# AnyLoc/Revisit-Anything

Measured on AMD Instinct MI355X. Metric: query_images_per_sec, higher is better.
Workload: dtype f32

## Files before the change

### revisit-anything_amd/csrc/api.hip

```cpp
#include <stdarg.h>
#include <stdlib.h>
#include <string.h>

#include <cmath>
#include <mutex>
#include <utility>

#include <initializer_list>

#include "ctx.h"

int segvlad_ctx::fail(int code, const char* fmt, ...) {
  va_list ap;
  va_start(ap, fmt);
  vsnprintf(err, sizeof(err), fmt, ap);
  va_end(ap);
  return code;
}

bool sv_is_device_ptr(const void* p) {
  hipPointerAttribute_t a;
  memset(&a, 0, sizeof(a));
  hipError_t e = hipPointerGetAttributes(&a, p);
  if (e != hipSuccess) {
// ... 97 lines not shown

int sv_fork_side(segvlad_ctx* ctx) {
  if (!ctx->side) {
    SV_HIP(hipStreamCreateWithFlags(&ctx->side, hipStreamNonBlocking));
    SV_HIP(hipEventCreateWithFlags(&ctx->ev_fork, hipEventDisableTiming));
    SV_HIP(hipEventCreateWithFlags(&ctx->ev_join, hipEventDisableTiming));
  }
  SV_HIP(hipEventRecord(ctx->ev_fork, ctx->stream));
  SV_HIP(hipStreamWaitEvent(ctx->side, ctx->ev_fork, 0));
  return SEGVLAD_OK;
}

int sv_join_side(segvlad_ctx* ctx) {
  SV_HIP(hipEventRecord(ctx->ev_join, ctx->side));
  SV_HIP(hipStreamWaitEvent(ctx->stream, ctx->ev_join, 0));
  return SEGVLAD_OK;
}

int sv_guard_check(segvlad_ctx* ctx) {
  if (!ctx->guard) return SEGVLAD_OK;
  SV_HIP(hipDeviceSynchronize());
  if (!ctx->guard_hit[0]) {
    ctx->for_each_buf([&](DevBuf& b) {
      if (!b.raw || ctx->guard_hit[0]) return;
      const int front = guard_words_hit(b.raw), back = guard_words_hit(static_cast<unsigned char*>(b.p) + b.fence_off());
      if (front)
        snprintf(ctx->guard_hit, sizeof(ctx->guard_hit), "%s: %d words written BELOW the buffer", b.tag, front);
      else if (back)
        snprintf(ctx->guard_hit, sizeof(ctx->guard_hit), "%s: %d words written beyond the %zu bytes requested", b.tag, back, b.fixed ? b.cap : b.req);
    });
  }
  if (ctx->guard_hit[0]) return ctx->fail(SEGVLAD_ERR_STATE, "guard: out-of-bounds write, buffer %s", ctx->guard_hit);
  return SEGVLAD_OK;
}

StageTimer* sv_stage_open(segvlad_ctx* c, const char* name, int* slot) {
  if (!c->profiling || c->scope_mute) return nullptr;
  StageTimer* t = &c->timers[name];
  if (t->used * 2 >= (int)t->ev.size()) {
    hipEvent_t a = nullptr, b = nullptr;
    (void)hipEventCreate(&a);
    (void)hipEventCreate(&b);
    t->ev.push_back(a);
    t->ev.push_back(b);
  }
  *slot = t->used++;
  (void)hipEventRecord(t->ev[2 * *slot], c->stream);
  return t;
}

hipError_t sv_max_dyn_lds(const void* fn, size_t bytes) {
  static std::mutex mu;
  static std::map<std::pair<int, const void*>, size_t> done;
  int dev = 0;
  hipError_t e = hipGetDevice(&dev);
  if (e != hipSuccess) return e;
  std::lock_guard<std::mutex> lk(mu);
  auto it = done.find({dev, fn});
  if (it != done.end() && it->second >= bytes) return hipSuccess;
  e = hipFuncSetAttribute(fn, hipFuncAttributeMaxDynamicSharedMemorySize, (int)bytes);
  if (e == hipSuccess) done[{dev, fn}] = bytes;
  return e;
}

extern "C" {

int segvlad_version(void) { return 300; }

int segvlad_create(segvlad_ctx** out, int device_id) {
  if (!out) return SEGVLAD_ERR_ARG;
  *out = nullptr;
  int ndev = 0;
  if (hipGetDeviceCount(&ndev) != hipSuccess || device_id < 0 || device_id >= ndev) return SEGVLAD_ERR_HIP;
  if (hipSetDevice(device_id) != hipSuccess) return SEGVLAD_ERR_HIP;
  segvlad_ctx* c = new (std::nothrow) segvlad_ctx();
  if (!c) return SEGVLAD_ERR_NOMEM;
  c->device = device_id;
  static const char* const env_keys[][2] = {{"SEGVLAD_KNN_FILTER", "knn_filter"},   {"SEGVLAD_F16_CFG", "f16_cfg"},
                                            {"SEGVLAD_F16_GM", "f16_gm"},           {"SEGVLAD_X3_TILE", "x3_tile"},
                                            {"SEGVLAD_X3_GM", "x3_gm"},             {"SEGVLAD_SEARCH_STATS", "search_stats"},
                                            {"SEGVLAD_ASSIGN_NARROW", "assign_narrow"}, {"SEGVLAD_DEBUG_SEARCH", "debug_search"},
                                            {"SEGVLAD_AGG_KPB", "agg_kpb"},
                                            {"SEGVLAD_KNN_HEURISTIC", "knn_heuristic"}, {"SEGVLAD_PCA_PATH", "pca_path"},
                                            {"SEGVLAD_COVER_ROWS", "cover_rows"}};
  for (auto& kv : env_keys)
    if (const char* v = getenv(kv[0])) (void)segvlad_set_option(c, kv[1], v);
#define SV_TAG_P(n) c->n.tag = #n; c->n.fixed = true;
#define SV_TAG_S(n) c->n.tag = #n;
  SV_PERSISTENT_BUFS(SV_TAG_P)
  SV_SCRATCH_BUFS(SV_TAG_S)
#undef SV_TAG_P
#undef SV_TAG_S
  if (const char* v = getenv("SEGVLAD_GUARD")) {
    if (v[0] && v[0] != '0') {
      c->guard = true;
      c->for_each_buf([](DevBuf& b) { b.guard = true; });
    }
  }
  if (const char* v = getenv("SEGVLAD_RCCL_LIB")) snprintf(sv_rccl_lib_override, sizeof(sv_rccl_lib_override), "%s", v);
  if (getenv("SEGVLAD_KNN_FP32")) (void)segvlad_set_option(c, "knn_filter", "fp32");
  if (getenv("SEGVLAD_PCA_FP32")) (void)segvlad_set_option(c, "pca_arith", "fp32");
  c->err[0] = 0;
  *out = c;
  return SEGVLAD_OK;
}

int segvlad_set_option(segvlad_ctx* ctx, const char* key, const char* value) {
  if (!ctx) return SEGVLAD_ERR_ARG;
  if (!key || !value) return ctx->fail(SEGVLAD_ERR_ARG, "set_option: null key/value");
  SvOptions& o = ctx->opt;
  auto as_int = [&](int* dst) -> int {
    char* end = nullptr;
    const long v = strtol(value, &end, 10);
    if (end == value || *end) return ctx->fail(SEGVLAD_ERR_ARG, "set_option(%s): '%s' is not an integer", key, value);
    *dst = (int)v;
    return SEGVLAD_OK;
  };
  if (!strcmp(key, "knn_filter")) {
    if (!strcmp(value, "auto")) o.knn_filter = 0;
    else if (!strcmp(value, "f16")) o.knn_filter = 1;
    else if (!strcmp(value, "bf16x3")) o.knn_filter = 2;
    else if (!strcmp(value, "fp32")) o.knn_filter = 3;
    else return ctx->fail(SEGVLAD_ERR_ARG, "set_option(knn_filter): want auto|f16|bf16x3|fp32, got '%s'", value);
    return SEGVLAD_OK;
  }
  if (!strcmp(key, "pca_arith")) {
    if (!strcmp(value, "auto") || !strcmp(value, "f16x3")) o.pca_fp32 = 0;
    else if (!strcmp(value, "fp32")) o.pca_fp32 = 1;
    else return ctx->fail(SEGVLAD_ERR_ARG, "set_option(pca_arith): want auto|f16x3|fp32, got '%s'", value);
    return SEGVLAD_OK;
  }
  if (!strcmp(key, "pca_path")) {
    if (!strcmp(value, "auto")) o.pca_path = 0;
    else if (!strcmp(value, "planes")) o.pca_path = 1;
    else if (!strcmp(value, "project")) o.pca_path = 2;
    else return ctx->fail(SEGVLAD_ERR_ARG, "set_option(pca_path): want auto|planes|project, got '%s'", value);
    return SEGVLAD_OK;
  }
  if (!strcmp(key, "vlad_assign")) {
    if (!strcmp(value, "hard")) {
      o.vlad_soft_temp = 0.f, o.vlad_soft_pooled = 0;
      return SEGVLAD_OK;
    }
    const int pooled = !strncmp(value, "soft_pooled:", 12);
    if (pooled || !strncmp(value, "soft:", 5)) {
      const char* t = value + (pooled ? 12 : 5);
      bool decimal = *t != 0 && (*t == '.' || (*t >= '0' && *t <= '9'));
      for (const char* c = t; *c && decimal; ++c) decimal = strchr("0123456789.eE+-", *c) != nullptr;
      char* end = nullptr;
      const float temp = decimal ? strtof(t, &end) : 0.f;
      if (decimal && end != t && *end == 0 && std::isfinite(temp) && temp > 0.f) {
        o.vlad_soft_temp = temp, o.vlad_soft_pooled = pooled;
        return SEGVLAD_OK;
      }
    }
    return ctx->fail(SEGVLAD_ERR_ARG, "set_option(vlad_assign): want hard|soft:<T>|soft_pooled:<T> with a finite decimal T > 0, got '%s'", value);
  }
  if (!strcmp(key, "vlad_burst")) {
    if (!strcmp(value, "off")) {
      o.vlad_burst = 0, o.burst_a = o.burst_b = o.burst_p = 0.f;
      return SEGVLAD_OK;
    }
    static const float lo[3] = {0.f, -8.f, 0.f}, hi[3] = {64.f, 16.f, 2.f};
    float v[3] = {0.f, 0.f, 0.f};
    const char* t = value;
    bool ok = true;
    for (int f = 0; f < 3 && ok; ++f) {
      const char* stop = f < 2 ? strchr(t, ':') : t + strlen(t);
      ok = stop != nullptr && stop != t && (*t == '.' || *t == '-' || (*t >= '0' && *t <= '9'));
      for (const char* c = t; ok && c < stop; ++c) ok = strchr("0123456789.eE+-", *c) != nullptr;
      if (!ok) break;
      char* end = nullptr;
      v[f] = strtof(t, &end);
      ok = end == stop && std::isfinite(v[f]) && v[f] >= lo[f] && v[f] <= hi[f];
      t = stop + 1;
    }
    if (ok) {
      o.vlad_burst = 1, o.burst_a = v[0], o.burst_b = v[1], o.burst_p = v[2];
      return SEGVLAD_OK;
    }
    return ctx->fail(SEGVLAD_ERR_ARG, "set_option(vlad_burst): want off|<a>:<b>:<p>, finite decimals with 0 <= a <= 64, -8 <= b <= 16, "
                                      "0 <= p <= 2, got '%s'", value);
  }
  if (!strcmp(key, "vlad_burst_scope")) {
    if (!strcmp(value, "image")) return o.burst_segment = 0, SEGVLAD_OK;
    if (!strcmp(value, "segment")) return o.burst_segment = 1, SEGVLAD_OK;
    return ctx->fail(SEGVLAD_ERR_ARG, "set_option(vlad_burst_scope): want image|segment, got '%s'", value);
  }
  auto as_dev = [&](int* dst, std::initializer_list<int> product_values, std::initializer_list<int> probe_values = {}) -> int {
    int v = *dst;
    SV_TRY(as_int(&v));
    bool ok = false;
    for (int a : product_values) ok = ok || a == v;
#ifdef SEGVLAD_ABLATIONS
    for (int a : probe_values) ok = ok || a == v;
#else
    (void)probe_values;
#endif
    if (!ok)
      return ctx->fail(SEGVLAD_ERR_ARG, "set_option(%s=%d): a development switch -- this library holds the default kernels only "
                       "(SEGVLAD_BUILD_ABLATIONS=1 builds lib/libsegvlad_hip_abl.so with the probes of csrc/segvlad_dev.h)", key, v);
    *dst = v;
    return SEGVLAD_OK;
  };
  if (!strcmp(key, "f16_cfg")) return as_dev(&o.f16_cfg, {-1, 250, 300, 62, 63}, {93, 94, 95});
  if (!strcmp(key, "f16_gm")) return as_int(&o.f16_gm);
  if (!strcmp(key, "f16_walk")) return as_int(&o.f16_walk);
  if (!strcmp(key, "f16_deep_cfg")) return as_dev(&o.f16_deep_cfg, {-1, 4, 5});
  if (!strcmp(key, "f16_buf")) return as_dev(&o.f16_buf, {-1, 0});
  if (!strcmp(key, "tnk_gram")) return as_int(&o.tnk_gram);
  if (!strcmp(key, "tnk_fork")) return as_int(&o.tnk_fork);
  if (!strcmp(key, "x3_tile")) return as_int(&o.x3_tile);
  if (!strcmp(key, "x3_gm")) return as_int(&o.x3_gm);
  if (!strcmp(key, "search_stats")) return as_int(&o.search_stats);
  if (!strcmp(key, "knn_heuristic")) return as_int(&o.knn_heuristic);
  if (!strcmp(key, "assign_narrow")) return as_int(&o.assign_narrow);
  if (!strcmp(key, "agg_kpb")) return as_int(&o.agg_kpb);
  if (!strcmp(key, "pj_nw")) return as_int(&o.pj_nw);
  if (!strcmp(key, "pj_f16")) return as_int(&o.pj_f16);
  if (!strcmp(key, "cover_rows")) return as_int(&o.cover_rows);
  if (!strcmp(key, "pj_planes")) return as_int(&o.pj_planes);
  if (!strcmp(key, "small_plan")) return as_int(&o.small_plan);
  if (!strcmp(key, "small_tail")) return as_int(&o.small_tail);
  if (!strcmp(key, "small_head")) return as_int(&o.small_head);
  if (!strcmp(key, "batch_l0_f16")) return as_int(&o.batch_l0_f16);
  if (!strcmp(key, "level_carry")) return as_int(&o.level_carry);
  if (!strcmp(key, "f16_persist_wgs")) return as_int(&o.f16_persist_wgs);
  if (!strcmp(key, "debug_small_tail")) return as_int(&o.debug_small_tail);
  if (!strcmp(key, "refine_group")) return as_int(&o.refine_group);
  if (!strcmp(key, "query_group")) return as_int(&o.query_group);
  if (!strcmp(key, "group_fetch")) return as_int(&o.group_fetch);
  if (!strcmp(key, "debug_search")) return as_int(&o.debug_search);
  if (!strcmp(key, "debug_fail_search")) return as_int(&o.debug_fail_search);
  if (!strcmp(key, "guard_undersize")) {
    if (!ctx->guard) return ctx->fail(SEGVLAD_ERR_STATE, "set_option(guard_undersize): the context was not created under SEGVLAD_GUARD=1");
    const char* colon = strchr(value, ':');
    bool found = false;
    ctx->for_each_buf([&](DevBuf& b) {
      if (!colon) b.shrink = 0;
      else if (strlen(b.tag) == (size_t)(colon - value) && !strncmp(b.tag, value, (size_t)(colon - value))) {
        b.shrink = atoi(colon + 1);
        found = true;
      }
    });
    if (colon && !found) return ctx->fail(SEGVLAD_ERR_ARG, "set_option(guard_undersize): no buffer named like '%s'", value);
    return SEGVLAD_OK;
  }
  return ctx->fail(SEGVLAD_ERR_ARG, "set_option: unknown key '%s'", key);
}

int segvlad_destroy(segvlad_ctx* ctx) {
  if (!ctx) return SEGVLAD_OK;
  (void)hipSetDevice(ctx->device);
  (void)hipStreamSynchronize(ctx->stream);
  sv_comm_release(ctx);
  if (ctx->side) {
    (void)hipStreamSynchronize(ctx->side);
    (void)hipStreamDestroy(ctx->side);
    (void)hipEventDestroy(ctx->ev_fork);
    (void)hipEventDestroy(ctx->ev_join);
  }
  if (ctx->h_pin) {
    (void)hipHostFree(ctx->h_pin);
    (void)hipEventDestroy(ctx->ev_scalars);
  }
  if (ctx->h_desc) (void)hipHostFree(ctx->h_desc);
  if (ctx->ev_desc) (void)hipEventDestroy(ctx->ev_desc);
  ctx->for_each_buf([](DevBuf& b) { b.release(); });
  for (auto& kv : ctx->timers)
    for (hipEvent_t e : kv.second.ev)
      if (e) (void)hipEventDestroy(e);
  delete ctx;
  return SEGVLAD_OK;
}

const char* segvlad_last_error(const segvlad_ctx* ctx) { return ctx ? ctx->err : "null context"; }

int segvlad_set_stream(segvlad_ctx* ctx, void* hip_stream) {
  if (!ctx) return SEGVLAD_ERR_ARG;
  ctx->stream = reinterpret_cast<hipStream_t>(hip_stream);
  return SEGVLAD_OK;
}

int segvlad_synchronize(segvlad_ctx* ctx) {
  CHECK_CTX();
  SV_HIP(hipStreamSynchronize(ctx->stream));
  return sv_guard_check(ctx);
}

int segvlad_set_profiling(segvlad_ctx* ctx, int on) {
  if (!ctx) return SEGVLAD_ERR_ARG;
  ctx->profiling = on != 0;
  return SEGVLAD_OK;
}

int segvlad_profile_reset(segvlad_ctx* ctx) {
  if (!ctx) return SEGVLAD_ERR_ARG;
  for (auto& kv : ctx->timers) {
    kv.second.used = 0;
    kv.second.launches = 0;
  }
  return SEGVLAD_OK;
}

// ... 285 lines not shown
```

### revisit-anything_amd/csrc/ctx.h

```cpp
#pragma once
#include <hip/hip_runtime.h>
#include <math.h>
#include <stdint.h>
#include <stdio.h>
#include <string.h>

#include <map>
#include <string>
#include <vector>

#include "../../include/segvlad.h"

#define SV_HIP(expr)                                                                              \
  do {                                                                                            \
    hipError_t _e = (expr);                                                                       \
    if (_e != hipSuccess) {                                                                       \
      return ctx->fail(SEGVLAD_ERR_HIP, "%s failed: %s (%s:%d)", #expr, hipGetErrorString(_e),    \
                       __FILE__, __LINE__);                                                       \
    }                                                                                             \
  } while (0)

#define SV_TRY(expr)          \
  do {                        \
    int _r = (expr);          \
// ... 27 lines not shown
  int e;
  frexpf(bound, &e);
  return ldexpf(1.f, 14 - e);
}

constexpr size_t SV_GUARD_BYTES = 1024;
constexpr uint32_t SV_GUARD_WORD = 0xA5C3F00Du;
struct DevBuf {
  void* p = nullptr;
  size_t cap = 0;
  const char* tag = "";
  bool guard = false;
  bool fixed = false;
  void* raw = nullptr;
  size_t req = 0;
  int shrink = 0;
  hipError_t reserve(size_t bytes) {
    if (guard) return reserve_guarded(bytes);
    if (bytes <= cap) return hipSuccess;
    if (p) {
      hipError_t e = hipFree(p);
      if (e != hipSuccess) return e;
      p = nullptr;
      cap = 0;
    }
    size_t want = bytes + bytes / 8 + 256;
    hipError_t e = hipMalloc(&p, want);
    if (e != hipSuccess) return e;
    cap = want;
    return hipSuccess;
  }
  hipError_t reserve_guarded(size_t bytes);
  size_t fence_off() const { return fixed ? cap : ((req > (size_t)shrink ? req - (size_t)shrink : 0) + 3) & ~(size_t)3; }
  void release() {
    if (raw) (void)hipFree(raw);
    else if (p) (void)hipFree(p);
    raw = nullptr;
    p = nullptr;
    cap = 0;
    req = 0;
  }
  template <class T>
  T* as() { return reinterpret_cast<T*>(p); }
};

struct StageTimer {
  std::vector<hipEvent_t> ev;
  int used = 0;
  int launches = 0;
};

struct SvOptions {
  int knn_filter = 0;
  int pca_fp32 = 0;
  int f16_cfg = -1;
  int f16_gm = -1;
  int f16_walk = -1;
  int f16_persist_wgs = 32;
  int f16_deep_cfg = -1;
  int f16_buf = -1;
  int tnk_gram = 1;
  int tnk_fork = 1;
  int x3_tile = 0;
  int x3_gm = -1;
  int search_stats = 0;
  int knn_heuristic = 1;
  int assign_narrow = 0;
  int agg_kpb = 4;
  int debug_fail_search = 0;
  int debug_search = 0;
  int debug_small_tail = 0;
  int batch_l0_f16 = 1;
  int level_carry = 1;
  int small_head = 1;
  int small_tail = 1;
  int small_plan = 1;
  int pj_f16 = 1;
  int pj_nw = 8;
  int refine_group = 1;
  int query_group = 0;
  int pca_path = 0;
  int cover_rows = 1;
  int pj_planes = 1;
  float vlad_soft_temp = 0.f;
  int vlad_soft_pooled = 0;
  int vlad_burst = 0;
  float burst_a = 0.f, burst_b = 0.f, burst_p = 0.f;
  int burst_segment = 0;
  int group_fetch = 0;
};

constexpr int SV_F16_KBLOCK = 1024;
inline int sv_f16_kblock(const SvOptions& o, int d) {
  if (o.f16_cfg == 300) return SV_F16_KBLOCK;
  return (o.f16_cfg < 0 && d >= 4096) ? SV_F16_KBLOCK : 0;
}
constexpr int SV_F16_KFLUSH = 64;
int sv_f16_eps_kblock(const SvOptions& o, int d);
inline bool sv_f16_bias_possible(const SvOptions& o, int64_t nq) { return nq > 128 && (o.f16_cfg < 0 || o.f16_cfg == 250 || o.f16_cfg == 300); }
enum class F16Kernel {
  None, BatchDefault, BatchComplement, BatchSmall, BatchUnbiased, BatchUnbiasedSmall, DeepFlush, DeepFlushComplement, DeepBlockedBuf, DeepBlocked,
  DeepBlockedBufComplement, DeepBlockedComplement, DeepUnbiased, OneImage64, OneImage128,
#ifdef SEGVLAD_ABLATIONS
  ProbePhases, ProbeNoEpilogue, ProbeNoEpilogueNoDma,
#endif
};
struct F16Choice {
  F16Kernel kernel;
  const char* why;
};
F16Choice sv_choose_f16_kernel(const SvOptions& o, bool bias_ok, int M, int64_t n_rows, int d, int b_stride, int skip);
inline float sv_f16_c_eps(int d, int kb, float bias_mult) {
  const float acc = kb > 0 ? (2.f * (float)kb + (float)((d + kb - 1) / kb) + 1.f) / 16777216.f : 2.f * (float)d / 16777216.f;
  return 2.5f * (1.f / 1024.f + 1.f / 4194304.f + bias_mult * acc);
}

struct SvSearchStats {
  int64_t levels = 0;
  int64_t filter = 0;
  int64_t n_fallback = 0;
  int64_t cand_max = 0;
  int64_t cand_sum = 0;
  int64_t refine_max = 0;
  int64_t refine_sum = 0;
  int64_t n_queries = 0;
  int64_t n_redo = 0;
  int64_t n_refine2 = 0;
  int64_t grp_groups = 0;
  int64_t grp_union_sum = 0;
  int64_t carry_rows = 0;
};

struct OpenDescribe {
  bool open = false;
  bool side_pending = false;
  int B = 0, S_tot = 0;
  StageTimer* timer = nullptr;
  int slot = 0;
};

struct segvlad_ctx {
  int device = 0;
  hipStream_t stream = nullptr;
  hipStream_t side = nullptr;
  hipEvent_t ev_fork = nullptr, ev_join = nullptr;
  uint32_t* h_pin = nullptr;
  hipEvent_t ev_scalars = nullptr;
  unsigned char* h_desc = nullptr;
  size_t h_desc_cap = 0;
  hipEvent_t ev_desc = nullptr;
  OpenDescribe desc;
  char err[512] = {0};
  bool profiling = false;
  bool scope_mute = false;
  std::map<std::string, StageTimer> timers;
  SvOptions opt;
  SvSearchStats sstats;

  int K = 0, D = 0, Kpad = 0;
  float vocab_maxabs = 0.f;
  float vocab_norm_max = 0.f;
  int P = 0, KD = 0, whiten = 0;
  float pca_w_scale = 0.f, pca_mean_maxabs = 0.f;
  bool pca_cproj_valid = false;
  int db_d = 0;
  int64_t db_n = 0;
// ... 315 lines not shown
```

### revisit-anything_amd/csrc/refine_group_kernels.hip

```cpp
#include "ctx.h"
#include "group_tile_dev.h"
#include "knn_dev.h"

namespace {

constexpr int RG_GMAX = 64;

constexpr int RG_UT = 1024;
__global__ __launch_bounds__(RG_UT) void refine_union_kernel(const uint32_t* __restrict__ ref_cnt, const uint32_t* __restrict__ ref_id,
                                                           int rcap, int m, int G, int d, int force, int ucap, int tcap ,
                                                           uint32_t* __restrict__ grp_cnt,
                                                           uint32_t* __restrict__ grp_ids, uint32_t* __restrict__ perrow,
                                                           uint32_t* __restrict__ work ,
                                                           uint16_t* __restrict__ grp_pos ,
                                                           const uint32_t* __restrict__ only_rows ) {
  extern __shared__ __attribute__((aligned(16))) unsigned char smem[];
  uint32_t* buf = reinterpret_cast<uint32_t*>(smem);
  __shared__ uint32_t off[RG_GMAX + 1];
  __shared__ uint32_t wtot[RG_UT / 64];
  const int b = blockIdx.x, tid = threadIdx.x, l = tid & 63, w = tid >> 6;
  const int q0 = b * G;
  const int nrows = min(G, m - q0);
  if (only_rows && !only_rows[q0]) {
    if (tid == 0) grp_cnt[b] = 0u;
// ... 25 lines not shown
        const uint32_t id = ref_id[(size_t)(q0 + t) * rcap + j];
        uint32_t h = (id * 2654435761u) & mask;
        for (;;) {
          const uint32_t prev = atomicCAS(&buf[h], 0xffffffffu, id);
          if (prev == 0xffffffffu || prev == id) break;
          h = (h + 1u) & mask;
        }
      }
    }
    __syncthreads();
    uint32_t base = 0;
    for (int j0 = 0; j0 < tcap; j0 += RG_UT) {
      const int j = j0 + tid;
      const uint32_t v = buf[j];
      const bool have = v != 0xffffffffu;
      const uint64_t mk = __builtin_amdgcn_ballot_w64(have);
      if (l == 0) wtot[w] = (uint32_t)__popcll(mk);
      __syncthreads();
      uint32_t o = base, all = 0;
      for (int x = 0; x < RG_UT / 64; ++x) {
        if (x < w) o += wtot[x];
        all += wtot[x];
      }
      const uint32_t pos = o + __builtin_amdgcn_mbcnt_hi((uint32_t)(mk >> 32), __builtin_amdgcn_mbcnt_lo((uint32_t)mk, 0u));
      if (have && pos < (uint32_t)ucap) uniq[pos] = v;
      base += all;
      __syncthreads();
    }
    U = (int)base;
    if (U <= ucap) {
      int np2 = 64;
      while (np2 < U) np2 <<= 1;
      for (int j = U + tid; j < np2; j += RG_UT) uniq[j] = 0xffffffffu;
      sv_bitonic<uint32_t, RG_UT>(uniq, np2, tid);
      for (int j = tid; j < U; j += RG_UT) grp_ids[(size_t)b * ucap + j] = uniq[j];
    }
    const float dd = (float)d * (1.f / 1024.f);
    const float cost_grp = (float)((U + 127) >> 7) * 8192.f * 0.038f * dd + 1.5f * (float)total * 0.022f;
    const float cost_row = (float)total * 0.39f * dd + (float)nrows * 21.f;
    grouped = U <= ucap && (force || cost_grp < cost_row);
    if (grouped) {
      for (int t = w; t < nrows; t += RG_UT / 64) {
        const int c = (int)(off[t + 1] - off[t]);
        for (int j = l; j < c; j += 64) {
          const uint32_t id = ref_id[(size_t)(q0 + t) * rcap + j];
          int lo = 0, hi = U;
          while (lo < hi) {
            const int mid = (lo + hi) >> 1;
            if (uniq[mid] < id) lo = mid + 1;
            else hi = mid;
          }
          grp_pos[(size_t)(q0 + t) * rcap + j] = (uint16_t)lo;
        }
      }
    }
  }
  if (tid == 0) {
    grp_cnt[b] = grouped ? (uint32_t)U : 0u;
    if (grouped) {
      const uint32_t nt = (uint32_t)(U + 127) >> 7;
      const uint32_t at = atomicAdd(&work[0], nt);
      for (uint32_t t = 0; t < nt; ++t) work[1 + at + t] = ((uint32_t)b << 5) | t;
    }
  }
  if (tid < nrows) perrow[q0 + tid] = grouped ? 0u : 1u;
}

template <int MT>
__global__ __launch_bounds__(256) void refine_group_gemm_kernel(const float* __restrict__ Q, const float* __restrict__ R, int d, int m,
                                                                int G, const float* __restrict__ qn, const float* __restrict__ rn,
                                                                const uint32_t* __restrict__ grp_cnt,
                                                                const uint32_t* __restrict__ grp_ids, int ucap,
                                                                uint64_t* __restrict__ keys, const uint32_t* __restrict__ work) {
  extern __shared__ __attribute__((aligned(16))) unsigned char smem[];
  float* tile = reinterpret_cast<float*>(smem);
  uint32_t* ids = reinterpret_cast<uint32_t*>(smem + sv_group_tile_bytes(MT));
  if (blockIdx.x >= work[0]) return;
  const uint32_t item = work[1 + blockIdx.x];
  const int b = (int)(item >> 5), c0 = (int)(item & 31u) * 128;
  const int U = (int)grp_cnt[b];
  const int tid = threadIdx.x, w = tid >> 6, l = tid & 63, i = l & 31, kk = l >> 5;
  const int q0 = b * G;
  const int q_end = min(q0 + G, m);
  if (tid < 128) ids[tid] = grp_ids[(size_t)b * ucap + (c0 + tid < U ? c0 + tid : 0)];
  __syncthreads();
  const SvGroupTileQ<MT> qrows = sv_group_tile_query_rows<MT>(Q, d, q0, q_end);
  f32x16 acc[MT];
  sv_group_tile_dots<MT>(tile, ids, qrows, R, d, acc);
  const int col = c0 + 32 * w + i;
  if (col < U) {
    const uint32_t id = ids[32 * w + i];
    const float r2 = rn[id];
#pragma unroll
    for (int t = 0; t < MT; ++t)
#pragma unroll
      for (int r = 0; r < 16; ++r) {
        const int q = q0 + 32 * t + sv_frag_row(r, kk);
        if (q < q_end) keys[(size_t)q * ucap + col] = ((uint64_t)f2key_(sv_d2(qn[q], r2, acc[t][r])) << 32) | id;
      }
  }
}

__global__ __launch_bounds__(256) void refine_group_select_kernel(const uint32_t* __restrict__ grp_cnt, const uint64_t* __restrict__ keys,
                                                                  const uint32_t* __restrict__ ref_cnt,
                                                                  const uint16_t* __restrict__ grp_pos, int rcap, int G, int ucap, int k,
                                                                  float* __restrict__ d2_out, int64_t* __restrict__ idx_out) {
  extern __shared__ __attribute__((aligned(16))) unsigned char smem[];
  uint64_t* a = reinterpret_cast<uint64_t*>(smem);
  const int64_t row = blockIdx.x;
  const int tid = threadIdx.x;
  if (grp_cnt[row / G] == 0) return;
  int n = (int)ref_cnt[row];
  if (n > rcap) n = 0;
  int np2 = 2;
  while (np2 < n) np2 <<= 1;
  for (int j = tid; j < np2; j += 256) a[j] = j < n ? keys[(size_t)row * ucap + grp_pos[(size_t)row * rcap + j]] : ~0ull;
  sv_bitonic<uint64_t>(a, np2, tid);
  for (int j = tid; j < k; j += 256) {
    float dd = INFINITY;
    int64_t id = -1;
    if (j < n) {
      dd = key2f_((uint32_t)(a[j] >> 32));
      id = (int64_t)(uint32_t)a[j];
    }
    d2_out[row * k + j] = dd;
    idx_out[row * k + j] = id;
  }
}

}

static int rg_group_rows(const segvlad_ctx* ctx) {
  const int h = ctx->opt.query_group;
  return (h >= 1 && h <= RG_GMAX) ? h : 32;
}

int sv_launch_refine_grouped(segvlad_ctx* ctx, const float* Q, const float* R, int nq, int d, const float* qn, const float* rn,
                             const uint32_t* ref_cnt, const uint32_t* ref_id, int rcap, int k, float* d2_out, int64_t* idx_out,
                             int* launches, const uint32_t* only_rows, int live_groups_hint) {
  if (launches) *launches = 0;
  if (nq <= 0) return SEGVLAD_OK;
  const int ucap = SV_RG_UCAP;
  const int G = only_rows ? 1 : rg_group_rows(ctx);
  int tcap = 1024;
  while (tcap < 32768 && 3 * (int64_t)tcap < 4 * (int64_t)G * rcap) tcap <<= 1;
  const bool can = ctx->opt.refine_group != 0 && d % SV_GT_KS == 0 && nq > 128 && (rcap <= 4096 || only_rows) &&
                   (reinterpret_cast<uintptr_t>(Q) & 15) == 0 && (reinterpret_cast<uintptr_t>(R) & 15) == 0;
  if (!can) {
    if (launches) *launches = 1;
    return sv_launch_refine_exact(ctx, Q, R, nq, d, qn, rn, ref_cnt, ref_id, rcap, k, d2_out, idx_out, only_rows);
  }
  const int nb = (nq + G - 1) / G;
  SV_HIP(ctx->s_grp_cnt.reserve((size_t)nb * 4));
  SV_HIP(ctx->s_grp_ids.reserve((size_t)nb * ucap * 4));
  SV_HIP(ctx->s_grp_rows.reserve((size_t)nq * 4));
  SV_HIP(ctx->s_grp_keys.reserve((size_t)nq * ucap * 8));
  SV_HIP(ctx->s_grp_pos.reserve((size_t)nq * rcap * 2));
  uint32_t* gcnt = ctx->s_grp_cnt.as<uint32_t>();
  uint32_t* gids = ctx->s_grp_ids.as<uint32_t>();
  uint32_t* prow = ctx->s_grp_rows.as<uint32_t>();
  uint64_t* gkeys = ctx->s_grp_keys.as<uint64_t>();
  static_assert(SV_RG_UCAP / 128 <= 32, "a work item holds its tile in 5 bits");
  const int max_items = ((live_groups_hint > 0 && live_groups_hint < nb) ? live_groups_hint : nb) * (ucap / 128);
  SV_HIP(ctx->s_grp_work.reserve((size_t)(max_items + 1) * 4));
  uint32_t* work = ctx->s_grp_work.as<uint32_t>();
  SV_HIP(hipMemsetAsync(work, 0, 4, ctx->stream));
  const size_t ulds = ((size_t)tcap + (size_t)ucap + RG_UT) * 4;
  if (ulds + 1024 > 64 * 1024) SV_HIP(sv_max_dyn_lds(reinterpret_cast<const void*>(refine_union_kernel), ulds));
  hipLaunchKernelGGL(refine_union_kernel, dim3(nb), dim3(RG_UT), ulds, ctx->stream, ref_cnt, ref_id, rcap, nq, G, d,
                     (ctx->opt.refine_group == 2 || only_rows) ? 1 : 0, ucap, tcap, gcnt, gids, prow, work, ctx->s_grp_pos.as<uint16_t>(), only_rows);
  SV_HIP(hipGetLastError());
  {
    const int mt = G > 32 ? 2 : 1;
    const size_t glds = sv_group_tile_bytes(mt) + 128 * 4;
    auto gk = mt == 2 ? refine_group_gemm_kernel<2> : refine_group_gemm_kernel<1>;
    SV_HIP(sv_max_dyn_lds(reinterpret_cast<const void*>(gk), glds));
    hipLaunchKernelGGL(gk, dim3(max_items), dim3(256), glds, ctx->stream, Q, R, d, nq, G, qn, rn, gcnt, gids, ucap, gkeys, work);
    SV_HIP(hipGetLastError());
  }
  {
    int rpad = 2;
    while (rpad < rcap) rpad <<= 1;
    if ((size_t)rpad * 8 + 1024 > 64 * 1024) SV_HIP(sv_max_dyn_lds(reinterpret_cast<const void*>(refine_group_select_kernel), (size_t)rpad * 8));
    hipLaunchKernelGGL(refine_group_select_kernel, dim3(nq), dim3(256), (size_t)rpad * 8, ctx->stream, gcnt, gkeys, ref_cnt,
                       ctx->s_grp_pos.as<uint16_t>(), rcap, G, ucap, k, d2_out, idx_out);
    SV_HIP(hipGetLastError());
  }
  if (launches) *launches = 4;
  return sv_launch_refine_exact(ctx, Q, R, nq, d, qn, rn, ref_cnt, ref_id, rcap, k, d2_out, idx_out, prow);
}

int sv_refine_group_stats(segvlad_ctx* ctx, int nq, int64_t* groups, int64_t* grouped, int64_t* union_sum) {
  const int nb = (nq + rg_group_rows(ctx) - 1) / rg_group_rows(ctx);
  std::vector<uint32_t> h(nb);
  SV_HIP(hipStreamSynchronize(ctx->stream));
  SV_HIP(hipMemcpy(h.data(), ctx->s_grp_cnt.p, (size_t)nb * 4, hipMemcpyDeviceToHost));
  int64_t g = 0, s = 0;
  for (uint32_t c : h) {
    if (c) ++g;
    s += c;
  }
  *groups = nb;
  *grouped = g;
  *union_sum = s;
  return SEGVLAD_OK;
}
```

### revisit-anything_amd/csrc/vlad_kernels.hip

```cpp
#include <stdio.h>
#include <stdlib.h>

#include "ctx.h"
#include "incidence_dev.h"
#include "mfma_f32_dev.h"

__global__ void vocab_norm_kernel(const float* __restrict__ C, int K, int D, float* __restrict__ inv) {
  const int k = blockIdx.x;
  float s = 0.f;
  for (int d = threadIdx.x; d < D; d += blockDim.x) {
    float v = C[(size_t)k * D + d];
    s = fmaf(v, v, s);
  }
  __shared__ float red[256];
  red[threadIdx.x] = s;
  __syncthreads();
  for (int o = 128; o > 0; o >>= 1) {
    if (threadIdx.x < o) red[threadIdx.x] += red[threadIdx.x + o];
    __syncthreads();
  }
  if (threadIdx.x == 0) inv[k] = 1.0f / fmaxf(sqrtf(red[0]), 1e-12f);
}

__global__ void vocab_bt_kernel(const float* __restrict__ C, const float* __restrict__ inv, int K, int D, int NT,
// ... 502 lines not shown
  __shared__ float ssum[128];
  const int gx = (N + 127) / 128;
  const int per = (int)((gridDim.x + 7) / 8);
  const int logical = (int)(blockIdx.x & 7) * per + (int)(blockIdx.x >> 3);
  if (logical >= gx * B) return;
  const int b = logical / gx, t0 = (logical - b * gx) * 128;
  const int tid = threadIdx.x, w = tid >> 6, l = tid & 63, i = l & 31, kk = l >> 5;
  const float* Tb = T + (size_t)b * D * N;
  const int lr = tid >> 5, lq = tid & 31;
  const int tl0 = t0 + 4 * lq;
  const int nvalid = N - tl0;
  f32x16 acc[NT];
#pragma unroll
  for (int n = 0; n < NT; ++n)
#pragma unroll
    for (int r = 0; r < 16; ++r) acc[n][r] = 0.f;
  float ss = 0.f;
  const int nch = D / DC;
  float4 va[4], vb[4];
#define SV_LOAD_CHUNK(V, c)                                                           \
  _Pragma("unroll") for (int j = 0; j < 4; ++j) {                                     \
    const float* p = Tb + (size_t)((c) * DC + lr + 8 * j) * N + tl0;                  \
    if (nvalid >= 4) {                                                                \
      const f32x4u u = *reinterpret_cast<const f32x4u*>(p);                           \
      V[j] = make_float4(u[0], u[1], u[2], u[3]);                                     \
    } else {                                                                          \
      V[j] = make_float4(nvalid > 0 ? p[0] : 0.f, nvalid > 1 ? p[1] : 0.f, nvalid > 2 ? p[2] : 0.f, 0.f); \
    }                                                                                 \
  }
#define SV_PARK_CHUNK(V, buf)                                                         \
  _Pragma("unroll") for (int j = 0; j < 4; ++j) {                                     \
    const int d_ = lr + 8 * j;                                                        \
    float* q = tile + (buf) * (DC * TS) + d_ * TS + ((4 * lq + rot(d_)) & 127);       \
    *reinterpret_cast<float4*>(q) = V[j];                                             \
  }
  SV_LOAD_CHUNK(va, 0)
  SV_PARK_CHUNK(va, 0)
  if (1 < nch) { SV_LOAD_CHUNK(va, 1) }
  __syncthreads();
#define SV_ASSIGN_STEP(c, VNEXT, VFREE)                                               \
  {                                                                                   \
    if ((c) + 2 < nch) { SV_LOAD_CHUNK(VFREE, (c) + 2) }                              \
    assign_wide_chunk<NT>(tile + ((c) & 1) * (DC * TS), bt, Xt, b, N, D, t0, tid, w, l, i, kk, (c), acc, ss);  \
    if ((c) + 1 < nch) { SV_PARK_CHUNK(VNEXT, ((c) + 1) & 1) }                        \
    __syncthreads();                                                                  \
  }
  for (int c = 0; c < nch; c += 2) {
    SV_ASSIGN_STEP(c, va, vb)
    if (c + 1 < nch) SV_ASSIGN_STEP(c + 1, vb, va)
  }
#undef SV_ASSIGN_STEP
#undef SV_LOAD_CHUNK
#undef SV_PARK_CHUNK
  constexpr int KP = NT * 32;
  float* sc = tile;
  ss += __shfl_xor(ss, 32);
  if (kk == 0) ssum[32 * w + i] = ss;
#pragma unroll
  for (int n = 0; n < NT; ++n)
#pragma unroll
    for (int r = 0; r < 16; ++r) sc[(32 * w + sv_frag_row(r, kk)) * (KP + 1) + n * 32 + i] = acc[n][r];
  __syncthreads();
  if (tid < 128 && t0 + tid < N) {
    const float rn = 1.0f / fmaxf(sqrtf(ssum[tid]), 1e-12f);
    float best = -INFINITY, second = -INFINITY;
    int bi = 0;
    for (int k = 0; k < K; ++k) {
      const float sv = sc[tid * (KP + 1) + k];
      if (sv > best) {
        second = best;
        best = sv;
        bi = k;
      } else if (sv > second) {
        second = sv;
      }
    }
    const size_t o = (size_t)b * N + t0 + tid;
    labels[o] = (uint8_t)bi;
    rnorm[o] = rn;
    if (gap) gap[o] = (K > 1) ? (best - second) * rn : INFINITY;
  }
}

int sv_launch_assign(segvlad_ctx* ctx, const float* tokens, int B, int N, float* xt, uint8_t* labels, float* rnorm,
                     float* gap) {
  const int NT = ctx->Kpad / 32;
  dim3 grid((N + 63) / 64, B), block(256);
  const float* bt = ctx->vocab_bt.as<float>();
  if (NT <= 2 && ctx->D % 32 == 0 && !ctx->opt.assign_narrow) {
    const unsigned tiles_total = (unsigned)((N + 127) / 128) * (unsigned)B;
    dim3 gridw((tiles_total + 7) / 8 * 8, 1);
    if (NT == 1)
      hipLaunchKernelGGL(assign_wide_kernel<1>, gridw, block, 0, ctx->stream, tokens, N, ctx->D, ctx->K, bt, xt, labels, rnorm, gap, B);
    else
      hipLaunchKernelGGL(assign_wide_kernel<2>, gridw, block, 0, ctx->stream, tokens, N, ctx->D, ctx->K, bt, xt, labels, rnorm, gap, B);
    SV_HIP(hipGetLastError());
    return SEGVLAD_OK;
  }
  switch (NT) {
    case 1:
      hipLaunchKernelGGL(assign_kernel<1>, grid, block, 0, ctx->stream, tokens, N, ctx->D, ctx->K, bt, xt, labels, rnorm, gap);
      break;
    case 2: {
#ifdef SEGVLAD_ABLATIONS
      const char* ab = getenv("SEGVLAD_ASSIGN_ABL");
      const int a = ab ? atoi(ab) : 0;
      if (a == 1) {
        hipLaunchKernelGGL((assign_kernel<2, 1>), grid, block, 0, ctx->stream, tokens, N, ctx->D, ctx->K, bt, xt, labels, rnorm, gap);
        break;
      } else if (a == 2) {
        hipLaunchKernelGGL((assign_kernel<2, 2>), grid, block, 0, ctx->stream, tokens, N, ctx->D, ctx->K, bt, xt, labels, rnorm, gap);
        break;
      } else if (a == 3) {
        hipLaunchKernelGGL((assign_kernel<2, 3>), grid, block, 0, ctx->stream, tokens, N, ctx->D, ctx->K, bt, xt, labels, rnorm, gap);
        break;
      }
#endif
      hipLaunchKernelGGL(assign_kernel<2>, grid, block, 0, ctx->stream, tokens, N, ctx->D, ctx->K, bt, xt, labels, rnorm, gap);
      break;
    }
    case 4:
      hipLaunchKernelGGL(assign_kernel<4>, grid, block, 0, ctx->stream, tokens, N, ctx->D, ctx->K, bt, xt, labels, rnorm, gap);
      break;
    default:
      return ctx->fail(SEGVLAD_ERR_LIMIT, "K=%d: supported cluster counts are 1..64 and 97..128 (Kpad in {32,64,128})", ctx->K);
  }
  SV_HIP(hipGetLastError());
  return SEGVLAD_OK;
}

__global__ __launch_bounds__(256) void prep_kernel(const uint8_t* __restrict__ labels, const uint64_t* __restrict__ inc,
                                                   const int32_t* __restrict__ seg_off,
                                                   const int64_t* __restrict__ adj_off, const uint8_t* __restrict__ adj,
                                                   int N, int K, int S_max, int SC, uint64_t* __restrict__ colmask,
                                                   float* __restrict__ gscale, int32_t* __restrict__ tok_order,
                                                   int32_t* __restrict__ lab_off, const float* __restrict__ rnorm,
                                                   float* __restrict__ rn_sorted, int stage, int ord_n,
                                                   int32_t* __restrict__ phys, int32_t* __restrict__ cov_cnt, int cover) {
  extern __shared__ __attribute__((aligned(16))) unsigned char smem[];
  const int b = blockIdx.x;
  const int nw = (N + 63) >> 6;
  const int s0 = seg_off[b], S = seg_off[b + 1] - s0;
  uint64_t* inc2 = reinterpret_cast<uint64_t*>(smem);
  uint64_t* lbits = inc2 + (size_t)S_max * nw;
  const int tid = threadIdx.x;
  if (adj && stage) {
    const int SW = (S_max + 63) >> 6;
    uint64_t* inc0 = reinterpret_cast<uint64_t*>(reinterpret_cast<int*>(lbits + (size_t)K * nw) + ord_n);
    uint64_t* nbr = inc0 + (size_t)S_max * nw;
    for (int idx = tid; idx < S * nw; idx += 256) inc0[idx] = inc[(size_t)s0 * nw + idx];
    for (int idx = tid; idx < S * SW; idx += 256) nbr[idx] = 0;
    __syncthreads();
    const uint8_t* a = adj + adj_off[b];
    for (int e = tid; e < S * S; e += 256)
      if (a[e]) {
        const int s = e / S, u = e - s * S;
        atomicOr(reinterpret_cast<unsigned long long*>(&nbr[s * SW + (u >> 6)]), 1ull << (u & 63));
      }
    __syncthreads();
    for (int idx = tid; idx < S * nw; idx += 256) {
      const int s = idx / nw, w = idx - s * nw;
      uint64_t v = 0;
      for (int uw = 0; uw < SW; ++uw) {
        uint64_t m = nbr[s * SW + uw];
        while (m) {
          const int u = (uw << 6) + __builtin_ctzll(m);
          m &= m - 1;
          v |= inc0[u * nw + w];
        }
      }
      inc2[idx] = v;
    }
  } else {
    for (int idx = tid; idx < S * nw; idx += 256) {
// ... 814 lines not shown
```

Before: 8953.

## Add double-buffered streaming assign kernel with register prefetch of token chunks

Adds a new assign kernel that streams the token matrix in 32-dim chunks. It prefetches the next two chunks into registers while MFMA runs on the current chunk, and double-buffers both the token and centroid chunks in LDS, with a rotated layout to avoid bank conflicts. The kernel is on by default when the wide-assign conditions hold, and it also writes the transposed Xt tile from LDS. Separately, the refine-group GEMM now stages query norms in LDS and loads the reference norm before the dot loop, removing scattered global reads from the epilogue. The costs are more register pressure and a more complex tail schedule.

```diff
diff --git a/revisit-anything_amd/csrc/api.hip b/revisit-anything_amd/csrc/api.hip
--- a/revisit-anything_amd/csrc/api.hip
+++ b/revisit-anything_amd/csrc/api.hip
@@ -203,7 +203,7 @@
                                             {"SEGVLAD_ASSIGN_NARROW", "assign_narrow"}, {"SEGVLAD_DEBUG_SEARCH", "debug_search"},
                                             {"SEGVLAD_AGG_KPB", "agg_kpb"},
                                             {"SEGVLAD_KNN_HEURISTIC", "knn_heuristic"}, {"SEGVLAD_PCA_PATH", "pca_path"},
-                                            {"SEGVLAD_COVER_ROWS", "cover_rows"}};
+                                            {"SEGVLAD_COVER_ROWS", "cover_rows"},   {"SEGVLAD_ASSIGN_STREAM", "assign_stream"}};
   for (auto& kv : env_keys)
     if (const char* v = getenv(kv[0])) (void)segvlad_set_option(c, kv[1], v);
 #define SV_TAG_P(n) c->n.tag = #n; c->n.fixed = true;
@@ -341,6 +341,7 @@
   if (!strcmp(key, "pj_f16")) return as_int(&o.pj_f16);
   if (!strcmp(key, "cover_rows")) return as_int(&o.cover_rows);
   if (!strcmp(key, "pj_planes")) return as_int(&o.pj_planes);
+  if (!strcmp(key, "assign_stream")) return as_dev(&o.assign_stream, {0, 1}, {2});
   if (!strcmp(key, "small_plan")) return as_int(&o.small_plan);
   if (!strcmp(key, "small_tail")) return as_int(&o.small_tail);
   if (!strcmp(key, "small_head")) return as_int(&o.small_head);
diff --git a/revisit-anything_amd/csrc/ctx.h b/revisit-anything_amd/csrc/ctx.h
--- a/revisit-anything_amd/csrc/ctx.h
+++ b/revisit-anything_amd/csrc/ctx.h
@@ -133,6 +133,7 @@
   int pca_path = 0;
   int cover_rows = 1;
   int pj_planes = 1;
+  int assign_stream = 1;
   float vlad_soft_temp = 0.f;
   int vlad_soft_pooled = 0;
   int vlad_burst = 0;
diff --git a/revisit-anything_amd/csrc/refine_group_kernels.hip b/revisit-anything_amd/csrc/refine_group_kernels.hip
--- a/revisit-anything_amd/csrc/refine_group_kernels.hip
+++ b/revisit-anything_amd/csrc/refine_group_kernels.hip
@@ -131,21 +131,29 @@
   const int tid = threadIdx.x, w = tid >> 6, l = tid & 63, i = l & 31, kk = l >> 5;
   const int q0 = b * G;
   const int q_end = min(q0 + G, m);
+  float* qns = reinterpret_cast<float*>(ids + 128);
   if (tid < 128) ids[tid] = grp_ids[(size_t)b * ucap + (c0 + tid < U ? c0 + tid : 0)];
+  else if (tid < 128 + 32 * MT) qns[tid - 128] = qn[min(q0 + tid - 128, q_end - 1)];
   __syncthreads();
+  const uint32_t id = ids[32 * w + i];
+  float r2 = rn[id];
   const SvGroupTileQ<MT> qrows = sv_group_tile_query_rows<MT>(Q, d, q0, q_end);
   f32x16 acc[MT];
   sv_group_tile_dots<MT>(tile, ids, qrows, R, d, acc);
   const int col = c0 + 32 * w + i;
+  asm volatile("" : "+v"(r2));
   if (col < U) {
-    const uint32_t id = ids[32 * w + i];
-    const float r2 = rn[id];
+    float q2[MT][16];
+#pragma unroll
+    for (int t = 0; t < MT; ++t)
+#pragma unroll
+      for (int r = 0; r < 16; ++r) q2[t][r] = qns[32 * t + sv_frag_row(r, kk)];
 #pragma unroll
     for (int t = 0; t < MT; ++t)
 #pragma unroll
       for (int r = 0; r < 16; ++r) {
         const int q = q0 + 32 * t + sv_frag_row(r, kk);
-        if (q < q_end) keys[(size_t)q * ucap + col] = ((uint64_t)f2key_(sv_d2(qn[q], r2, acc[t][r])) << 32) | id;
+        if (q < q_end) keys[(size_t)q * ucap + col] = ((uint64_t)f2key_(sv_d2(q2[t][r], r2, acc[t][r])) << 32) | id;
       }
   }
 }
@@ -221,7 +229,7 @@
   SV_HIP(hipGetLastError());
   {
     const int mt = G > 32 ? 2 : 1;
-    const size_t glds = sv_group_tile_bytes(mt) + 128 * 4;
+    const size_t glds = sv_group_tile_bytes(mt) + 128 * 4 + 32 * mt * 4;
     auto gk = mt == 2 ? refine_group_gemm_kernel<2> : refine_group_gemm_kernel<1>;
     SV_HIP(sv_max_dyn_lds(reinterpret_cast<const void*>(gk), glds));
     hipLaunchKernelGGL(gk, dim3(max_items), dim3(256), glds, ctx->stream, Q, R, d, nq, G, qn, rn, gcnt, gids, ucap, gkeys, work);
diff --git a/revisit-anything_amd/csrc/vlad_kernels.hip b/revisit-anything_amd/csrc/vlad_kernels.hip
--- a/revisit-anything_amd/csrc/vlad_kernels.hip
+++ b/revisit-anything_amd/csrc/vlad_kernels.hip
@@ -608,6 +608,167 @@
   }
 }
 
+template <int NT>
+__device__ __forceinline__ void assign_stream_mul(const float* __restrict__ tl, const float* __restrict__ cb, int w, int l, int i, int kk,
+                                                  f32x16 (&acc)[NT], float& ss) {
+  constexpr int DC = 32, TS = 128;
+  auto rot = [](int d) { return 8 * (d >> 2) + 32 * (d & 1); };
+#pragma unroll 8
+  for (int st = 0; st < DC / 2; ++st) {
+    const float x = tl[(2 * st + kk) * TS + ((32 * w + i + rot(2 * st + kk)) & 127)];
+    ss = fmaf(x, x, ss);
+#pragma unroll
+    for (int n = 0; n < NT; ++n) acc[n] = MFMA32(x, cb[(st * NT + n) * 64 + l], acc[n]);
+  }
+}
+
+__device__ __forceinline__ void assign_stream_xt(const float* __restrict__ tl, float* __restrict__ Xtile, int D, int tid, int last, int c) {
+  constexpr int DC = 32, TS = 128;
+#pragma unroll
+  for (int it = 0; it < 4; ++it) {
+    const int idx = it * 256 + tid;
+    const int tok = min(idx >> 3, last), c4 = idx & 7;
+    const float* q = tl + (4 * c4) * TS;
+    const int t_a = (tok + 8 * c4) & 127, t_b = (tok + 8 * c4 + 32) & 127;
+    const float4 o = make_float4(q[t_a], q[TS + t_b], q[2 * TS + t_a], q[3 * TS + t_b]);
+    *reinterpret_cast<float4*>(Xtile + (size_t)tok * D + c * DC + 4 * c4) = o;
+  }
+}
+
+template <int NT, int NCB>
+__global__ __launch_bounds__(256, NCB == 2 ? 3 : 4) void assign_stream_kernel(const float* __restrict__ T, int N, int D, int K,
+                                                            const float* __restrict__ bt, float* __restrict__ Xt,
+                                                            uint8_t* __restrict__ labels, float* __restrict__ rnorm,
+                                                            float* __restrict__ gap, int B) {
+  constexpr int DC = 32, TS = 128;
+  constexpr int KP = NT * 32;
+  constexpr int CEN = (DC / 2) * NT * 64;
+  constexpr int TOK = 2 * DC * TS;
+  static_assert(TOK + NCB * CEN >= 128 * (KP + 1) + 128, "the epilogue's scores and norms lie over the chunk buffers");
+  auto rot = [](int d) { return 8 * (d >> 2) + 32 * (d & 1); };
+  __shared__ __attribute__((aligned(16))) float lds[TOK + NCB * CEN];
+  float* tile = lds;
+  float* cen = lds + TOK;
+  const int gx = (N + 127) / 128;
+  const int per = (int)((gridDim.x + 7) / 8);
+  const int logical = (int)(blockIdx.x & 7) * per + (int)(blockIdx.x >> 3);
+  if (logical >= gx * B) return;
+  const int b = logical / gx, t0 = (logical - b * gx) * 128;
+  const int tid = threadIdx.x, w = tid >> 6, l = tid & 63, i = l & 31, kk = l >> 5;
+  const float* Tb = T + (size_t)b * D * N;
+  float* Xtile = Xt + ((size_t)b * N + t0) * D;
+  const int last = min(127, N - 1 - t0);
+  const int lr = tid >> 5, lq = tid & 31;
+  const int tl0 = t0 + 4 * lq;
+  const int cback = min(tl0, N - 4);
+  const int cfwd = min(tl0, N - 1);
+  const int sh = tl0 - cback;
+  const bool sh0 = sh == 0, sh1 = sh == 1, sh2 = sh == 2;
+  f32x16 acc[NT];
+#pragma unroll
+  for (int n = 0; n < NT; ++n)
+#pragma unroll
+    for (int r = 0; r < 16; ++r) acc[n][r] = 0.f;
+  float ss = 0.f;
+  const int nch = D / DC;
+  float4 va[4], vb[4], ca0, ca1 = make_float4(0.f, 0.f, 0.f, 0.f), cb0, cb1 = ca1;
+#define SV_LOAD_ROWS(V, c, J0)                                                        \
+  _Pragma("unroll") for (int j = (J0); j < 4; ++j) {                                  \
+    const f32x4u u = *reinterpret_cast<const f32x4u*>(Tb + ((ptrdiff_t)((c) * DC + lr + 8 * j) * N + cback)); \
+    V[j] = make_float4(u[0], u[1], u[2], u[3]);                                       \
+  }
+#define SV_LOAD_CEN(C0, C1, c)                                                        \
+  C0 = *reinterpret_cast<const float4*>(bt + (size_t)(c) * CEN + 4 * tid);            \
+  if (NT == 2) C1 = *reinterpret_cast<const float4*>(bt + (size_t)(c) * CEN + 4 * (tid + 256));
+#define SV_PARK_ROWS(V, buf, J0)                                                      \
+  _Pragma("unroll") for (int j = (J0); j < 4; ++j) {                                  \
+    const int d_ = lr + 8 * j;                                                        \
+    const float4 u = V[j];                                                            \
+    const float4 p = make_float4(sh0 ? u.x : sh1 ? u.y : sh2 ? u.z : u.w, sh0 ? u.y : sh1 ? u.z : u.w, sh0 ? u.z : u.w, u.w); \
+    *reinterpret_cast<float4*>(tile + (buf) * (DC * TS) + d_ * TS + ((4 * lq + rot(d_)) & 127)) = p; \
+  }
+#define SV_PARK_CEN(C0, C1, buf)                                                      \
+  *reinterpret_cast<float4*>(cen + (NCB == 2 ? (buf) : 0) * CEN + 4 * tid) = C0;      \
+  if (NT == 2) *reinterpret_cast<float4*>(cen + (NCB == 2 ? (buf) : 0) * CEN + 4 * (tid + 256)) = C1;
+  {
+    const f32x4u u = *reinterpret_cast<const f32x4u*>(Tb + ((size_t)lr * N + cfwd));
+    va[0] = make_float4(u[0], u[1], u[2], u[3]);
+  }
+  SV_LOAD_ROWS(va, 0, 1)
+  SV_LOAD_CEN(ca0, ca1, 0)
+  *reinterpret_cast<float4*>(tile + lr * TS + ((4 * lq + rot(lr)) & 127)) = va[0];
+  SV_PARK_ROWS(va, 0, 1)
+  SV_PARK_CEN(ca0, ca1, 0)
+  if (1 < nch) {
+    SV_LOAD_ROWS(va, 1, 0)
+    SV_LOAD_CEN(ca0, ca1, 1)
+  }
+  __syncthreads();
+#define SV_STREAM_STEP(c, VNEXT, CN0, CN1, VFREE, CF0, CF1, PRE1, PRE2)               \
+  {                                                                                   \
+    if (PRE2) {                                                                       \
+      SV_LOAD_ROWS(VFREE, (c) + 2, 0)                                                 \
+      SV_LOAD_CEN(CF0, CF1, (c) + 2)                                                   \
+    }                                                                                 \
+    assign_stream_mul<NT>(tile + ((c) & 1) * (DC * TS), cen + (NCB == 2 ? ((c) & 1) : 0) * CEN, w, l, i, kk, acc, ss); \
+    assign_stream_xt(tile + ((c) & 1) * (DC * TS), Xtile, D, tid, last, (c));         \
+    if (NCB == 1 && (PRE1)) __syncthreads();                                          \
+    if (PRE1) {                                                                       \
+      SV_PARK_ROWS(VNEXT, ((c) + 1) & 1, 0)                                           \
+      SV_PARK_CEN(CN0, CN1, ((c) + 1) & 1)                                             \
+    }                                                                                 \
+    __syncthreads();                                                                  \
+  }
+  int c = 0;
+  for (; c + 3 < nch; c += 2) {
+    SV_STREAM_STEP(c, va, ca0, ca1, vb, cb0, cb1, 1, 1)
+    SV_STREAM_STEP(c + 1, vb, cb0, cb1, va, ca0, ca1, 1, 1)
+  }
+  if (nch - c == 3) {
+    SV_STREAM_STEP(c, va, ca0, ca1, vb, cb0, cb1, 1, 1)
+    SV_STREAM_STEP(c + 1, vb, cb0, cb1, va, ca0, ca1, 1, 0)
+    SV_STREAM_STEP(c + 2, va, ca0, ca1, vb, cb0, cb1, 0, 0)
+  } else if (nch - c == 2) {
+    SV_STREAM_STEP(c, va, ca0, ca1, vb, cb0, cb1, 1, 0)
+    SV_STREAM_STEP(c + 1, vb, cb0, cb1, va, ca0, ca1, 0, 0)
+  } else {
+    SV_STREAM_STEP(c, va, ca0, ca1, vb, cb0, cb1, 0, 0)
+  }
+#undef SV_STREAM_STEP
+#undef SV_LOAD_ROWS
+#undef SV_LOAD_CEN
+#undef SV_PARK_ROWS
+#undef SV_PARK_CEN
+  float* sc = lds;
+  float* ssum = lds + 128 * (KP + 1);
+  ss += __shfl_xor(ss, 32);
+  if (kk == 0) ssum[32 * w + i] = ss;
+#pragma unroll
+  for (int n = 0; n < NT; ++n)
+#pragma unroll
+    for (int r = 0; r < 16; ++r) sc[(32 * w + sv_frag_row(r, kk)) * (KP + 1) + n * 32 + i] = acc[n][r];
+  __syncthreads();
+  if (tid < 128 && t0 + tid < N) {
+    const float rn = 1.0f / fmaxf(sqrtf(ssum[tid]), 1e-12f);
+    float best = -INFINITY, second = -INFINITY;
+    int bi = 0;
+    for (int k = 0; k < K; ++k) {
+      const float sv = sc[tid * (KP + 1) + k];
+      if (sv > best) {
+        second = best;
+        best = sv;
+        bi = k;
+      } else if (sv > second) {
+        second = sv;
+      }
+    }
+    const size_t o = (size_t)b * N + t0 + tid;
+    labels[o] = (uint8_t)bi;
+    rnorm[o] = rn;
+    if (gap) gap[o] = (K > 1) ? (best - second) * rn : INFINITY;
+  }
+}
+
 int sv_launch_assign(segvlad_ctx* ctx, const float* tokens, int B, int N, float* xt, uint8_t* labels, float* rnorm,
                      float* gap) {
   const int NT = ctx->Kpad / 32;
@@ -616,6 +777,24 @@
   if (NT <= 2 && ctx->D % 32 == 0 && !ctx->opt.assign_narrow) {
     const unsigned tiles_total = (unsigned)((N + 127) / 128) * (unsigned)B;
     dim3 gridw((tiles_total + 7) / 8 * 8, 1);
+    if (ctx->opt.assign_stream) {
+#ifdef SEGVLAD_ABLATIONS
+      if (ctx->opt.assign_stream == 2) {
+        if (NT == 1)
+          hipLaunchKernelGGL((assign_stream_kernel<1, 1>), gridw, block, 0, ctx->stream, tokens, N, ctx->D, ctx->K, bt, xt, labels, rnorm, gap, B);
+        else
+          hipLaunchKernelGGL((assign_stream_kernel<2, 1>), gridw, block, 0, ctx->stream, tokens, N, ctx->D, ctx->K, bt, xt, labels, rnorm, gap, B);
+        SV_HIP(hipGetLastError());
+        return SEGVLAD_OK;
+      }
+#endif
+      if (NT == 1)
+        hipLaunchKernelGGL((assign_stream_kernel<1, 2>), gridw, block, 0, ctx->stream, tokens, N, ctx->D, ctx->K, bt, xt, labels, rnorm, gap, B);
+      else
+        hipLaunchKernelGGL((assign_stream_kernel<2, 2>), gridw, block, 0, ctx->stream, tokens, N, ctx->D, ctx->K, bt, xt, labels, rnorm, gap, B);
+      SV_HIP(hipGetLastError());
+      return SEGVLAD_OK;
+    }
     if (NT == 1)
       hipLaunchKernelGGL(assign_wide_kernel<1>, gridw, block, 0, ctx->stream, tokens, N, ctx->D, ctx->K, bt, xt, labels, rnorm, gap, B);
     else
```

After: 9022 (median of 6 runs). About the same (+0.8%).
